# OmerMersin/video-stab

Hardware: AMD Instinct MI355X
Metric: stabilized frames/sec @1080p (whole job; warp-stage HBM GB/s in roofline) (higher is better)
Workload: dtype u8

## Files before the change

video-stab_amd/csrc/k_lk.hip:

```cpp
#include "vs_common.h"

namespace vsd {
namespace {

constexpr int MAX_LEVELS = 8;

struct LKArgs {
    LKLevel levels[MAX_LEVELS];
    int max_level;
    const float* prev_pts;
    float* next_pts;
    uint8_t* status;
    float* err;
    int n;
    const int32_t* d_n;
    int win;
    int max_count;
    double eps2;
};

template <int CTRL>
__device__ __forceinline__ int dpp_mov(int v) {
    return __builtin_amdgcn_update_dpp(0, v, CTRL, 0xF, 0xF, true);
}
__device__ __forceinline__ int wave_sum_i32(int v) {
    v += dpp_mov<0xB1>(v);
    v += dpp_mov<0x4E>(v);
    v += dpp_mov<0x141>(v);
    v += dpp_mov<0x140>(v);
    return __builtin_amdgcn_readlane(v, 0) + __builtin_amdgcn_readlane(v, 16) +
           __builtin_amdgcn_readlane(v, 32) + __builtin_amdgcn_readlane(v, 48);
}
template <int CTRL>
__device__ __forceinline__ long long dpp_mov64(long long v) {
    const int lo = dpp_mov<CTRL>((int)(unsigned)(unsigned long long)v);
    const int hi = dpp_mov<CTRL>((int)((unsigned long long)v >> 32));
    return (long long)(((unsigned long long)(unsigned)hi << 32) | (unsigned)lo);
}
__device__ __forceinline__ long long wave_sum(int p) {
    long long v = p;
    v += dpp_mov64<0xB1>(v);
    v += dpp_mov64<0x4E>(v);
    v += dpp_mov64<0x141>(v);
    v += dpp_mov64<0x140>(v);
    const int lo = (int)(unsigned)(unsigned long long)v, hi = (int)((unsigned long long)v >> 32);
    long long t = 0;
#pragma unroll
    for (int r = 0; r < 64; r += 16) {
        const unsigned l = (unsigned)__builtin_amdgcn_readlane(lo, r);
        const unsigned h = (unsigned)__builtin_amdgcn_readlane(hi, r);
        t += (long long)(((unsigned long long)h << 32) | l);
    }
    return t;
}

__device__ __forceinline__ int descale(int x, int n) { return (x + (1 << (n - 1))) >> n; }

struct Weights { int w00, w01, w10, w11; };

__device__ __forceinline__ Weights make_weights(float a, float b) {
    Weights w;
    w.w00 = f_round((1.f - a) * (1.f - b) * 16384.f);
    w.w01 = f_round(a * (1.f - b) * 16384.f);
    w.w10 = f_round((1.f - a) * b * 16384.f);
    w.w11 = 16384 - w.w00 - w.w01 - w.w10;
    return w;
}

typedef const __attribute__((address_space(1))) uint8_t* gmem_u8;
__device__ __forceinline__ gmem_u8 uniform_global(const uint8_t* p) {
    const unsigned long long v = (unsigned long long)p;
    const unsigned lo = (unsigned)__builtin_amdgcn_readfirstlane((int)(unsigned)v), hi = (unsigned)__builtin_amdgcn_readfirstlane((int)(unsigned)(v >> 32));
    return (gmem_u8)(((unsigned long long)hi << 32) | lo);
}

constexpr int LK_MARGIN = 6;
constexpr int LK_WIN_MAX = 31;



__device__ __forceinline__ void divmod_small(int i, int d, float inv_d, int& q, int& r) {
    q = (int)(((float)i + 0.5f) * inv_d);
    r = i - q * d;
}

template <int NPX>
__device__ __forceinline__ void lk_track(const LKArgs& a, const int pt) {
    constexpr int WM = NPX <= 4 ? 16 : (NPX <= 7 ? 21 : LK_WIN_MAX);
    constexpr int PWM = WM + 1, RWM = WM + 1 + 2 * LK_MARGIN;
    constexpr int DR = NPX <= 7 ? 3 : 5;
    constexpr int PPM = (PWM + 2 + 3) & ~3;
    constexpr int SRM = (PWM + 1 + 3) / 4, NGM = (PWM + DR - 1) / DR;
    static_assert(SRM * NGM <= 64, "one derivative round per level");
    constexpr int PN = (PPM * (PWM + 2) + 63) / 64, RN = (RWM * RWM + 63) / 64;
    constexpr int PBYTES = (PN * 64 > PPM * (NGM * DR + 2) + 4 ? PN * 64 : PPM * (NGM * DR + 2) + 4);
    __shared__ __attribute__((aligned(16))) uint8_t pI_[4 + PBYTES];
    uint8_t* const pI = pI_ + 4;
    __shared__ __attribute__((aligned(16))) short2 pD[(PWM + 1) * PPM];
    __shared__ uint8_t region[RN * 64];
    const int lane = threadIdx.x;
    int n = a.n;
    if (a.d_n) { int dn = *a.d_n; n = dn < n ? dn : n; }
    if (pt >= n) return;
    const int win = a.win, area = win * win;
    const int PW = win + 1, PP = (PW + 2 + 3) & ~3;
    const int RW = win + 1 + 2 * LK_MARGIN;
    const float inv_pp = 1.0f / (float)PP, inv_rw = 1.0f / (float)RW, inv_win = 1.0f / (float)win;
    uint32_t off[NPX];
#pragma unroll
    for (int k = 0; k < NPX; k++) {
        const int p = lane + 64 * k;
        int yy = 0, xx = 0;
        if (p < area) divmod_small(p, win, inv_win, yy, xx);
        off[k] = (uint32_t)((yy + 1) * PP + xx + 1) | ((uint32_t)(yy * RW + xx) << 16);
    }
#define LK_VALID(k) (lane + 64 * (k) < area)
#define LK_POFF(k) ((int)(off[k] & 0xFFFFu))
#define LK_ROFF(k) ((int)(off[k] >> 16))
    int p_y0, p_x0, p_sy, p_sx, r_y0, r_x0, r_sy, r_sx;
    divmod_small(lane, PP, inv_pp, p_y0, p_x0);
    divmod_small(64, PP, inv_pp, p_sy, p_sx);
    divmod_small(lane, RW, inv_rw, r_y0, r_x0);
    divmod_small(64, RW, inv_rw, r_sy, r_sx);
    const float halfWin = (win - 1) * 0.5f;
    const float FLT_SCALE = 1.f / (1 << 20);
    const float px0 = a.prev_pts[2 * pt], py0 = a.prev_pts[2 * pt + 1];
    float outx = 0.f, outy = 0.f;
    int status = 1;
    float err = 0.f;

    for (int level = a.max_level; level >= 0; level--) {
        const LKLevel L = a.levels[level];
        const float scale = (float)(1. / (double)(1 << level));
        float prevx = px0 * scale, prevy = py0 * scale;
        if (level == a.max_level) { outx = prevx; outy = prevy; }
        else { outx = outx * 2.f; outy = outy * 2.f; }
        prevx -= halfWin; prevy -= halfWin;
        const int ipx = f_floor(prevx), ipy = f_floor(prevy);
        if (ipx < -win || ipx >= L.w || ipy < -win || ipy >= L.h) {
            if (level == 0) { status = 0; err = 0.f; }
            continue;
        }
        float cx = outx - halfWin, cy = outy - halfWin;
        int rx0 = f_floor(cx) - LK_MARGIN, ry0 = f_floor(cy) - LK_MARGIN;
        __syncthreads();
        const int pcount = PP * (PW + 2);
        if (ipx >= 1 && ipy >= 1 && ipx - 1 + PP <= L.w && ipy + PW + 1 <= L.h) {
            const gmem_u8 pbase = uniform_global(L.prev + ((size_t)(ipy - 1) * L.stride + (ipx - 1)));
            constexpr int PB_ = 10;
            int y = p_y0, x = p_x0;
#pragma unroll
            for (int k0 = 0; k0 < PN; k0 += PB_) {
                uint8_t vI[PB_];
#pragma unroll
                for (int k = k0; k < k0 + PB_ && k < PN; k++) {
                    const bool ok = lane + 64 * k < pcount;
                    vI[k - k0] = pbase[ok ? (uint32_t)(y * (int)L.stride + x) : 0u];
                    x += p_sx; y += p_sy;
                    if (x >= PP) { x -= PP; y++; }
                }
#pragma unroll
                for (int k = k0; k < k0 + PB_ && k < PN; k++) pI[lane + 64 * k] = vI[k - k0];
                __builtin_amdgcn_sched_barrier(0);
            }
        } else {
            int y = p_y0, x = p_x0;
            for (int i = lane; i < pcount; i += 64) {
                const int X = ipx - 1 + x, Y = ipy - 1 + y;
                pI[i] = L.prev[(size_t)reflect101(Y, L.h) * L.stride + reflect101(X, L.w)];
                x += p_sx; y += p_sy;
                if (x >= PP) { x -= PP; y++; }
            }
        }
        auto stage_region = [&]() {
            const bool inside = rx0 >= 0 && ry0 >= 0 && rx0 + RW <= L.w && ry0 + RW <= L.h;
            int y = r_y0, x = r_x0;
            asm volatile("" : "+v"(x), "+v"(y));
            if (inside) {
                const gmem_u8 rbase = uniform_global(L.next + ((size_t)ry0 * L.stride + rx0));
                constexpr int RB_ = 10;
#pragma unroll
                for (int k0 = 0; k0 < RN; k0 += RB_) {
                    uint8_t vR[RB_];
#pragma unroll
                    for (int k = k0; k < k0 + RB_ && k < RN; k++) {
                        const bool ok = lane + 64 * k < RW * RW;
                        vR[k - k0] = rbase[ok ? (uint32_t)(y * (int)L.stride + x) : 0u];
                        x += r_sx; y += r_sy;
                        if (x >= RW) { x -= RW; y++; }
                    }
#pragma unroll
                    for (int k = k0; k < k0 + RB_ && k < RN; k++) region[lane + 64 * k] = vR[k - k0];
                    __builtin_amdgcn_sched_barrier(0);
                }
            } else {
                for (int i = lane; i < RW * RW; i += 64) {
                    const int X = rx0 + x, Y = ry0 + y;
                    region[i] = L.next[(size_t)reflect101(Y, L.h) * L.stride + reflect101(X, L.w)];
                    x += r_sx; y += r_sy;
                    if (x >= RW) { x -= RW; y++; }
                }
            }
        };
        stage_region();
        __syncthreads();
        {
            const int sr = (PW + 1 + 3) >> 2;
            int g, c;
            divmod_small(lane, sr, 1.0f / (float)sr, g, c);
            const int y = 1 + g * DR, x = 4 * c;
            if (y <= PW) {
                const bool masked = !(ipx >= 0 && ipy >= 0 && ipx + PW <= L.w && ipy + PW <= L.h);
                int t[3][6];
                auto load_row = [&](int j, int* tj) {
                    const uint32_t* q = reinterpret_cast<const uint32_t*>(pI + j * PP) + c;
                    const uint32_t lo = q[-1], mid = q[0], hi = q[1];
                    tj[0] = lo >> 24;
                    tj[1] = mid & 255u; tj[2] = (mid >> 8) & 255u; tj[3] = (mid >> 16) & 255u; tj[4] = mid >> 24;
                    tj[5] = hi & 255u;
                };
                load_row(y - 1, t[0]);
                load_row(y, t[1]);
#pragma unroll
                for (int r = 0; r < DR; r++) {
                    const int* t0 = t[r % 3];
                    const int* t1 = t[(r + 1) % 3];
                    int* t2 = t[(r + 2) % 3];
                    load_row(y + r + 1, t2);
                    int av[6], bv[6];
#pragma unroll
                    for (int k = 0; k < 6; k++) {
                        av[k] = (t0[k] + t2[k]) * 3 + t1[k] * 10;
                        bv[k] = t2[k] - t0[k];
                    }
                    uint32_t o[4];
#pragma unroll
                    for (int k = 0; k < 4; k++) {
                        const int dx = av[k + 2] - av[k], dy = (bv[k + 2] + bv[k]) * 3 + bv[k + 1] * 10;
                        o[k] = ((uint32_t)dx & 0xFFFFu) | ((uint32_t)dy << 16);
                        if (masked && ((unsigned)(ipx - 1 + x + k) >= (unsigned)L.w || (unsigned)(ipy - 1 + y + r) >= (unsigned)L.h)) o[k] = 0u;
                    }
                    if (y + r <= PW) *reinterpret_cast<uint4*>(&pD[(y + r) * PP + x]) = make_uint4(o[0], o[1], o[2], o[3]);
                    __builtin_amdgcn_sched_barrier(0);
                }
            }
        }
        __syncthreads();
#pragma unroll
        for (int k = 0; k < NPX; k++) asm volatile("" : "+v"(off[k]));
        Weights wt = make_weights(prevx - ipx, prevy - ipy);
        short Iw[NPX], Ix[NPX], Iy[NPX];
        int pA11 = 0, pA12 = 0, pA22 = 0;
#pragma unroll
        for (int k = 0; k < NPX; k++) {
            const int o = LK_POFF(k);
            int ival = descale(__mul24((int)pI[o], wt.w00) + __mul24((int)pI[o + 1], wt.w01) +
                               __mul24((int)pI[o + PP], wt.w10) + __mul24((int)pI[o + PP + 1], wt.w11), 9);
            const short2 d00 = pD[o], d01 = pD[o + 1], d10 = pD[o + PP], d11 = pD[o + PP + 1];
            int ixval = descale(__mul24((int)d00.x, wt.w00) + __mul24((int)d01.x, wt.w01) +
                                __mul24((int)d10.x, wt.w10) + __mul24((int)d11.x, wt.w11), 14);
            int iyval = descale(__mul24((int)d00.y, wt.w00) + __mul24((int)d01.y, wt.w01) +
                                __mul24((int)d10.y, wt.w10) + __mul24((int)d11.y, wt.w11), 14);
            if (!LK_VALID(k)) { ival = 0; ixval = 0; iyval = 0; }
            Iw[k] = (short)ival; Ix[k] = (short)ixval; Iy[k] = (short)iyval;
            pA11 += __mul24(ixval, ixval);
            pA12 += __mul24(ixval, iyval);
            pA22 += __mul24(iyval, iyval);
        }
        const long long sA11 = wave_sum(pA11), sA12 = wave_sum(pA12), sA22 = wave_sum(pA22);
        const float A11 = (float)sA11 * FLT_SCALE, A12 = (float)sA12 * FLT_SCALE, A22 = (float)sA22 * FLT_SCALE;
        float D = A11 * A22 - A12 * A12;
        const float minEig = (A22 + A11 - sqrtf((A11 - A22) * (A11 - A22) + 4.f * A12 * A12)) /
                             (float)(2 * win * win);
        if (minEig < 1e-4f || D < FLT_EPSILON) {
            if (level == 0) status = 0;
            continue;
        }
        D = 1.f / D;
        float pdx = 0.f, pdy = 0.f;
        for (int j = 0; j < a.max_count; j++) {
            const int inx = f_floor(cx), iny = f_floor(cy);
            if (inx < -win || inx >= L.w || iny < -win || iny >= L.h) {
                if (level == 0) status = 0;
                break;
            }
            wt = make_weights(cx - inx, cy - iny);
            int lx = inx - rx0, ly = iny - ry0;
            if (!(lx >= 0 && ly >= 0 && lx + win + 1 <= RW && ly + win + 1 <= RW)) {
                __syncthreads();
                rx0 = inx - LK_MARGIN; ry0 = iny - LK_MARGIN;
                stage_region();
                __syncthreads();
                lx = LK_MARGIN; ly = LK_MARGIN;
            }
            int pb1 = 0, pb2 = 0;
            {
                const int rbase = ly * RW + lx;
#pragma unroll
                for (int k = 0; k < NPX; k++) {
                    const uint8_t* r0 = &region[rbase + LK_ROFF(k)];
                    const int v = descale(__mul24((int)r0[0], wt.w00) + __mul24((int)r0[1], wt.w01) +
                                          __mul24((int)r0[RW], wt.w10) + __mul24((int)r0[RW + 1], wt.w11), 9);
                    const int diff = v - Iw[k];
                    pb1 += __mul24(diff, (int)Ix[k]);
                    pb2 += __mul24(diff, (int)Iy[k]);
                }
            }
            const long long sb1 = wave_sum(pb1), sb2 = wave_sum(pb2);
            const float b1 = (float)sb1 * FLT_SCALE, b2 = (float)sb2 * FLT_SCALE;
            const float dx = (A12 * b2 - A22 * b1) * D;
            const float dy = (A12 * b1 - A11 * b2) * D;
            cx += dx; cy += dy;
            outx = cx + halfWin; outy = cy + halfWin;
            if ((double)dx * (double)dx + (double)dy * (double)dy <= a.eps2) break;
            if (j > 0 && (double)fabsf(dx + pdx) < 0.01 && (double)fabsf(dy + pdy) < 0.01) {
                outx -= dx * 0.5f; outy -= dy * 0.5f;
                break;
            }
            pdx = dx; pdy = dy;
        }
        if (status && level == 0) {
            const float npx = outx - halfWin, npy = outy - halfWin;
            const int inx = f_floor(npx), iny = f_floor(npy);
            if (inx < -win || inx >= L.w || iny < -win || iny >= L.h) {
                status = 0;
            } else {
                wt = make_weights(npx - inx, npy - iny);
                int lx = inx - rx0, ly = iny - ry0;
                if (!(lx >= 0 && ly >= 0 && lx + win + 1 <= RW && ly + win + 1 <= RW)) {
                    __syncthreads();
                    rx0 = inx - LK_MARGIN; ry0 = iny - LK_MARGIN;
                    stage_region();
                    __syncthreads();
                    lx = LK_MARGIN; ly = LK_MARGIN;
                }
                int es = 0;
                {
                    const int rbase = ly * RW + lx;
#pragma unroll
                    for (int k = 0; k < NPX; k++) {
                        const uint8_t* r0 = &region[rbase + LK_ROFF(k)];
                        const int v = descale(__mul24((int)r0[0], wt.w00) + __mul24((int)r0[1], wt.w01) +
                                              __mul24((int)r0[RW], wt.w10) + __mul24((int)r0[RW + 1], wt.w11), 9);
                        const int diff = v - Iw[k];
                        es += LK_VALID(k) ? (diff < 0 ? -diff : diff) : 0;
                    }
                }
                const long long est = wave_sum(es);
                err = (float)est * 1.f / (float)(32 * win * win);
            }
        }
    }
#undef LK_VALID
#undef LK_POFF
#undef LK_ROFF
    if (lane == 0) {
        a.next_pts[2 * pt] = outx;
        a.next_pts[2 * pt + 1] = outy;
        a.status[pt] = (uint8_t)status;
        a.err[pt] = err;
    }
}

template <int NPX>
__global__ __launch_bounds__(64) void lk_kernel(LKArgs a) { lk_track<NPX>(a, blockIdx.x); }

template <int NPX>
__global__ __launch_bounds__(64) void lk_batch_kernel(const LKArgs* __restrict__ table) {
    lk_track<NPX>(table[blockIdx.y], blockIdx.x);
}

int fill_lk_args(LKArgs& a, const LKLevel* levels, int max_level, const float* d_prev_pts, int n, const int32_t* d_n,
                 float* d_next_pts, uint8_t* d_status, float* d_err, int win, int max_iters, double eps) {
    if (!levels || max_level < 0 || max_level >= MAX_LEVELS || n < 0 || win < 3 || win > 31 ||
        !d_prev_pts || !d_next_pts || !d_status || !d_err) {
        set_last_error("pyr_lk: invalid argument (3 <= win <= 31, max_level < 8)");
        return VS_ERR_INVALID_ARG;
    }
    for (int i = 0; i <= max_level; i++) a.levels[i] = levels[i];
    for (int i = max_level + 1; i < MAX_LEVELS; i++) a.levels[i] = levels[max_level];
    a.max_level = max_level;
    a.prev_pts = d_prev_pts; a.next_pts = d_next_pts; a.status = d_status; a.err = d_err;
    a.n = n; a.d_n = d_n; a.win = win;
    a.max_count = max_iters < 0 ? 0 : (max_iters > 100 ? 100 : max_iters);
    double e = eps < 0 ? 0. : (eps > 10. ? 10. : eps);
    a.eps2 = e * e;
    return VS_OK;
}

}

size_t lk_item_bytes() { return sizeof(LKArgs); }

int lk_fill_item(void* host_item, const LKLevel* levels, int max_level, const float* d_prev_pts, int n,
                 const int32_t* d_n, float* d_next_pts, uint8_t* d_status, float* d_err, int win, int max_iters,
                 double eps) {
    return fill_lk_args(*static_cast<LKArgs*>(host_item), levels, max_level, d_prev_pts, n, d_n, d_next_pts, d_status,
                        d_err, win, max_iters, eps);
}

int launch_pyr_lk_batch(const void* d_table, int items, int n_max, int win, hipStream_t st) {
    if (!d_table || items < 1 || items > 65535 || n_max < 0 || win < 3 || win > 31) {
        set_last_error("pyr_lk_batch: invalid argument");
        return VS_ERR_INVALID_ARG;
    }
    if (n_max == 0) return VS_OK;
    const LKArgs* t = static_cast<const LKArgs*>(d_table);
    const int npx = (win * win + 63) / 64;
    dim3 grid(n_max, items), block(64);
    if (npx <= 4) hipLaunchKernelGGL(lk_batch_kernel<4>, grid, block, 0, st, t);
    else if (npx <= 7) hipLaunchKernelGGL(lk_batch_kernel<7>, grid, block, 0, st, t);
    else hipLaunchKernelGGL(lk_batch_kernel<16>, grid, block, 0, st, t);
    VS_HIP_TRY(hipGetLastError());
    return VS_OK;
}

int launch_pyr_lk(const LKLevel* levels, int max_level, const float* d_prev_pts, int n,
                  const int32_t* d_n, float* d_next_pts, uint8_t* d_status, float* d_err, int win,
                  int max_iters, double eps, hipStream_t st) {
    LKArgs a;
    VS_TRY(fill_lk_args(a, levels, max_level, d_prev_pts, n, d_n, d_next_pts, d_status, d_err, win, max_iters, eps));
    if (n == 0) return VS_OK;
    const int npx = (win * win + 63) / 64;
    dim3 grid(n), block(64);
    if (npx <= 4) hipLaunchKernelGGL(lk_kernel<4>, grid, block, 0, st, a);
    else if (npx <= 7) hipLaunchKernelGGL(lk_kernel<7>, grid, block, 0, st, a);
    else hipLaunchKernelGGL(lk_kernel<16>, grid, block, 0, st, a);
    VS_HIP_TRY(hipGetLastError());
    return VS_OK;
}

int run_pyr_lk_op(const uint8_t* d_prev, const uint8_t* d_next, size_t stride, int w, int h,
                  const float* d_prev_pts, int n, float* d_next_pts, uint8_t* d_status,
                  float* d_err, int win, int max_level, int max_iters, double eps, hipStream_t st) {
    if (!d_prev || !d_next || w <= 0 || h <= 0 || max_level < 0 || max_level >= MAX_LEVELS) {
        set_last_error("pyr_lk: invalid argument");
        return VS_ERR_INVALID_ARG;
    }
    int lw[MAX_LEVELS], lh[MAX_LEVELS];
    int levels = 0;
    {
        int sw = w, sh = h;
        for (int level = 0; level <= max_level; level++) {
            lw[level] = sw; lh[level] = sh;
            levels = level;
            sw = (sw + 1) / 2; sh = (sh + 1) / 2;
            if (sw <= win || sh <= win) break;
        }
    }
    size_t img_bytes = 0;
    for (int i = 1; i <= levels; i++) img_bytes += (size_t)lw[i] * lh[i];
    uint8_t* scratch = nullptr;
    VS_HIP_TRY(hipMalloc((void**)&scratch, 2 * img_bytes + 64));
    LKLevel L[MAX_LEVELS];
    uint8_t* pp = scratch;
    uint8_t* pn = scratch + img_bytes;
    int rc = VS_OK;
    for (int i = 0; i <= levels && rc == VS_OK; i++) {
        L[i].w = lw[i]; L[i].h = lh[i];
        if (i == 0) { L[i].prev = d_prev; L[i].next = d_next; L[i].stride = stride; }
        else {
            rc = launch_pyr_down(L[i - 1].prev, L[i - 1].stride, lw[i - 1], lh[i - 1], pp, lw[i], st);
            if (rc == VS_OK) rc = launch_pyr_down(L[i - 1].next, L[i - 1].stride, lw[i - 1], lh[i - 1], pn, lw[i], st);
            L[i].prev = pp; L[i].next = pn; L[i].stride = lw[i];
            pp += (size_t)lw[i] * lh[i]; pn += (size_t)lw[i] * lh[i];
        }
    }
    if (rc == VS_OK) rc = launch_pyr_lk(L, levels, d_prev_pts, n, nullptr, d_next_pts, d_status, d_err, win, max_iters, eps, st);
    hipError_t e = hipStreamSynchronize(st);
    (void)hipFree(scratch);
    if (rc == VS_OK && e != hipSuccess) { set_last_error(hipGetErrorString(e)); rc = VS_ERR_HIP; }
    return rc;
}

}
```

Measured before the change: 127,400.

## Stage LK patches with aligned dword loads and packed 16-bit derivative math

Stages the prev patch and next search region from global memory with aligned 32-bit loads joined by alignbyte, replacing per-byte loads, and pads the region to a 4-byte pitch. The Scharr derivative computation now uses packed 16-bit SIMD arithmetic and perm/alignbit instead of scalar byte unpacking. Wave reductions do their first steps in 32-bit where the value range proves no overflow, and per-NPX VGPR limits are set on the kernels. Pyramid level buffers are padded to 4 bytes so the aligned path applies, at the cost of more complex staging code and register-pressure tuning risk.

```diff
diff --git a/video-stab_amd/csrc/k_lk.hip b/video-stab_amd/csrc/k_lk.hip
--- a/video-stab_amd/csrc/k_lk.hip
+++ b/video-stab_amd/csrc/k_lk.hip
@@ -1,4 +1,5 @@
 #include "vs_common.h"
+#include "lk_stage.h"
 
 namespace vsd {
 namespace {
@@ -31,18 +32,33 @@
     return __builtin_amdgcn_readlane(v, 0) + __builtin_amdgcn_readlane(v, 16) +
            __builtin_amdgcn_readlane(v, 32) + __builtin_amdgcn_readlane(v, 48);
 }
+constexpr long long LK_DIFF_MAX = 8161, LK_GRAD_MAX = 4081;
+constexpr long long LK_TERM_MAX = LK_DIFF_MAX * LK_GRAD_MAX;
+constexpr int lk_sum32_steps(int npx) {
+    int s = 0;
+    while (s < 4 && (long long)npx * LK_TERM_MAX * (2ll << s) <= 2147483647ll) s++;
+    return s;
+}
 template <int CTRL>
 __device__ __forceinline__ long long dpp_mov64(long long v) {
     const int lo = dpp_mov<CTRL>((int)(unsigned)(unsigned long long)v);
     const int hi = dpp_mov<CTRL>((int)((unsigned long long)v >> 32));
     return (long long)(((unsigned long long)(unsigned)hi << 32) | (unsigned)lo);
 }
+template <int NPX>
 __device__ __forceinline__ long long wave_sum(int p) {
+    constexpr int S32 = lk_sum32_steps(NPX);
+    static_assert((long long)NPX * LK_TERM_MAX <= 2147483647ll, "a lane's partial sum fits int32");
+    static_assert((long long)NPX * LK_TERM_MAX * (1ll << S32) <= 2147483647ll, "the 32-bit steps cannot overflow");
+    if (S32 >= 1) p += dpp_mov<0xB1>(p);
+    if (S32 >= 2) p += dpp_mov<0x4E>(p);
+    if (S32 >= 3) p += dpp_mov<0x141>(p);
+    if (S32 >= 4) p += dpp_mov<0x140>(p);
     long long v = p;
-    v += dpp_mov64<0xB1>(v);
-    v += dpp_mov64<0x4E>(v);
-    v += dpp_mov64<0x141>(v);
-    v += dpp_mov64<0x140>(v);
+    if (S32 < 1) v += dpp_mov64<0xB1>(v);
+    if (S32 < 2) v += dpp_mov64<0x4E>(v);
+    if (S32 < 3) v += dpp_mov64<0x141>(v);
+    if (S32 < 4) v += dpp_mov64<0x140>(v);
     const int lo = (int)(unsigned)(unsigned long long)v, hi = (int)((unsigned long long)v >> 32);
     long long t = 0;
 #pragma unroll
@@ -53,6 +69,12 @@
     }
     return t;
 }
+
+typedef unsigned short u16x2 __attribute__((ext_vector_type(2)));
+__device__ __forceinline__ uint32_t pk_add(uint32_t a, uint32_t b) { return __builtin_bit_cast(uint32_t, __builtin_bit_cast(u16x2, a) + __builtin_bit_cast(u16x2, b)); }
+__device__ __forceinline__ uint32_t pk_sub(uint32_t a, uint32_t b) { return __builtin_bit_cast(uint32_t, __builtin_bit_cast(u16x2, a) - __builtin_bit_cast(u16x2, b)); }
+__device__ __forceinline__ uint32_t pk_mul(uint32_t a, uint32_t b) { return __builtin_bit_cast(uint32_t, __builtin_bit_cast(u16x2, a) * __builtin_bit_cast(u16x2, b)); }
+__device__ __forceinline__ uint32_t pk_mad(uint32_t a, uint32_t b, uint32_t c) { return pk_add(pk_mul(a, b), c); }
 
 __device__ __forceinline__ int descale(int x, int n) { return (x + (1 << (n - 1))) >> n; }
 
@@ -68,6 +90,7 @@
 }
 
 typedef const __attribute__((address_space(1))) uint8_t* gmem_u8;
+typedef const __attribute__((address_space(1))) uint32_t* gmem_u32;
 __device__ __forceinline__ gmem_u8 uniform_global(const uint8_t* p) {
     const unsigned long long v = (unsigned long long)p;
     const unsigned lo = (unsigned)__builtin_amdgcn_readfirstlane((int)(unsigned)v), hi = (unsigned)__builtin_amdgcn_readfirstlane((int)(unsigned)(v >> 32));
@@ -93,18 +116,20 @@
     constexpr int SRM = (PWM + 1 + 3) / 4, NGM = (PWM + DR - 1) / DR;
     static_assert(SRM * NGM <= 64, "one derivative round per level");
     constexpr int PN = (PPM * (PWM + 2) + 63) / 64, RN = (RWM * RWM + 63) / 64;
+    constexpr int RPM = (RWM + 3) & ~3;
+    constexpr int PND = (PPM / 4 * (PWM + 2) + 63) / 64, RND = (RPM / 4 * RWM + 63) / 64;
     constexpr int PBYTES = (PN * 64 > PPM * (NGM * DR + 2) + 4 ? PN * 64 : PPM * (NGM * DR + 2) + 4);
     __shared__ __attribute__((aligned(16))) uint8_t pI_[4 + PBYTES];
     uint8_t* const pI = pI_ + 4;
     __shared__ __attribute__((aligned(16))) short2 pD[(PWM + 1) * PPM];
-    __shared__ uint8_t region[RN * 64];
+    __shared__ __attribute__((aligned(16))) uint8_t region[RPM * RWM];
     const int lane = threadIdx.x;
     int n = a.n;
     if (a.d_n) { int dn = *a.d_n; n = dn < n ? dn : n; }
     if (pt >= n) return;
     const int win = a.win, area = win * win;
     const int PW = win + 1, PP = (PW + 2 + 3) & ~3;
-    const int RW = win + 1 + 2 * LK_MARGIN;
+    const int RW = win + 1 + 2 * LK_MARGIN, RP = (RW + 3) & ~3;
     const float inv_pp = 1.0f / (float)PP, inv_rw = 1.0f / (float)RW, inv_win = 1.0f / (float)win;
     uint32_t off[NPX];
 #pragma unroll
@@ -112,16 +137,18 @@
         const int p = lane + 64 * k;
         int yy = 0, xx = 0;
         if (p < area) divmod_small(p, win, inv_win, yy, xx);
-        off[k] = (uint32_t)((yy + 1) * PP + xx + 1) | ((uint32_t)(yy * RW + xx) << 16);
+        off[k] = (uint32_t)((yy + 1) * PP + xx + 1) | ((uint32_t)(yy * RP + xx) << 16);
     }
 #define LK_VALID(k) (lane + 64 * (k) < area)
 #define LK_POFF(k) ((int)(off[k] & 0xFFFFu))
 #define LK_ROFF(k) ((int)(off[k] >> 16))
-    int p_y0, p_x0, p_sy, p_sx, r_y0, r_x0, r_sy, r_sx;
-    divmod_small(lane, PP, inv_pp, p_y0, p_x0);
-    divmod_small(64, PP, inv_pp, p_sy, p_sx);
-    divmod_small(lane, RW, inv_rw, r_y0, r_x0);
-    divmod_small(64, RW, inv_rw, r_sy, r_sx);
+    auto walk = [&](int d, float inv_d, int& y0, int& x0, int& sy, int& sx) {
+        int ln = lane;
+        asm volatile("" : "+v"(ln));
+        divmod_small(ln, d, inv_d, y0, x0);
+        divmod_small(64, d, inv_d, sy, sx);
+        return ln;
+    };
     const float halfWin = (win - 1) * 0.5f;
     const float FLT_SCALE = 1.f / (1 << 20);
     const float px0 = a.prev_pts[2 * pt], py0 = a.prev_pts[2 * pt + 1];
@@ -145,10 +172,33 @@
         int rx0 = f_floor(cx) - LK_MARGIN, ry0 = f_floor(cy) - LK_MARGIN;
         __syncthreads();
         const int pcount = PP * (PW + 2);
-        if (ipx >= 1 && ipy >= 1 && ipx - 1 + PP <= L.w && ipy + PW + 1 <= L.h) {
+        const bool p_inside = lk_box_inside(ipx - 1, ipy - 1, PP, PW + 2, L.w, L.h);
+        if (p_inside && (((unsigned long long)L.prev | (unsigned long long)L.stride) & 3u) == 0) {
+            const gmem_u8 pbase = uniform_global(L.prev + (size_t)(ipy - 1) * L.stride);
+            const int nd = PP >> 2, cnt = nd * (PW + 2), x0 = ipx - 1;
+            const LKStageSrc s0 = lk_stage_src(x0, PP, 0);
+            int y, j, sy, sj;
+            const int ln = walk(nd, 4.0f * inv_pp, y, j, sy, sj);
+            uint32_t vlo[PND], vhi[PND];
+#pragma unroll
+            for (int k = 0; k < PND; k++) {
+                const bool ok = ln + 64 * k < cnt;
+                const LKStageSrc sc = lk_stage_src(x0, PP, j);
+                const uint32_t row = (uint32_t)(y * (int)L.stride);
+                vlo[k] = *reinterpret_cast<gmem_u32>(pbase + (ok ? row + (uint32_t)sc.lo : (uint32_t)s0.lo));
+                vhi[k] = *reinterpret_cast<gmem_u32>(pbase + (ok ? row + (uint32_t)sc.hi : (uint32_t)s0.lo));
+                j += sj; y += sy;
+                if (j >= nd) { j -= nd; y++; }
+            }
+#pragma unroll
+            for (int k = 0; k < PND; k++)
+                if (ln + 64 * k < cnt) reinterpret_cast<uint32_t*>(pI)[ln + 64 * k] = lk_stage_join(vlo[k], vhi[k], s0.shift);
+            __builtin_amdgcn_sched_barrier(0);
+        } else if (p_inside) {
             const gmem_u8 pbase = uniform_global(L.prev + ((size_t)(ipy - 1) * L.stride + (ipx - 1)));
             constexpr int PB_ = 10;
-            int y = p_y0, x = p_x0;
+            int y, x, p_sy, p_sx;
+            walk(PP, inv_pp, y, x, p_sy, p_sx);
 #pragma unroll
             for (int k0 = 0; k0 < PN; k0 += PB_) {
                 uint8_t vI[PB_];
@@ -164,7 +214,8 @@
                 __builtin_amdgcn_sched_barrier(0);
             }
         } else {
-            int y = p_y0, x = p_x0;
+            int y, x, p_sy, p_sx;
+            walk(PP, inv_pp, y, x, p_sy, p_sx);
             for (int i = lane; i < pcount; i += 64) {
                 const int X = ipx - 1 + x, Y = ipy - 1 + y;
                 pI[i] = L.prev[(size_t)reflect101(Y, L.h) * L.stride + reflect101(X, L.w)];
@@ -173,30 +224,63 @@
             }
         }
         auto stage_region = [&]() {
-            const bool inside = rx0 >= 0 && ry0 >= 0 && rx0 + RW <= L.w && ry0 + RW <= L.h;
-            int y = r_y0, x = r_x0;
-            asm volatile("" : "+v"(x), "+v"(y));
-            if (inside) {
+            const bool inside = lk_box_inside(rx0, ry0, RW, RW, L.w, L.h);
+            if (inside && (((unsigned long long)L.next | (unsigned long long)L.stride) & 3u) == 0) {
+                const gmem_u8 rbase = uniform_global(L.next + (size_t)ry0 * L.stride);
+                const int nd = RP >> 2, cnt = nd * RW;
+                const LKStageSrc s0 = lk_stage_src(rx0, RW, 0);
+                int y, j, sy, sj;
+                const int ln = walk(nd, 1.0f / (float)nd, y, j, sy, sj);
+                constexpr int RB_ = 5;
+#pragma unroll
+                for (int k0 = 0; k0 < RND; k0 += RB_) {
+                    uint32_t vlo[RB_], vhi[RB_];
+#pragma unroll
+                    for (int k = k0; k < k0 + RB_ && k < RND; k++) {
+                        const bool ok = ln + 64 * k < cnt;
+                        const LKStageSrc sc = lk_stage_src(rx0, RW, j);
+                        const uint32_t row = (uint32_t)(y * (int)L.stride);
+                        vlo[k - k0] = *reinterpret_cast<gmem_u32>(rbase + (ok ? row + (uint32_t)sc.lo : (uint32_t)s0.lo));
+                        vhi[k - k0] = *reinterpret_cast<gmem_u32>(rbase + (ok ? row + (uint32_t)sc.hi : (uint32_t)s0.lo));
+                        j += sj; y += sy;
+                        if (j >= nd) { j -= nd; y++; }
+                    }
+#pragma unroll
+                    for (int k = k0; k < k0 + RB_ && k < RND; k++)
+                        if (ln + 64 * k < cnt)
+                            reinterpret_cast<uint32_t*>(region)[ln + 64 * k] = lk_stage_join(vlo[k - k0], vhi[k - k0], s0.shift);
+                    __builtin_amdgcn_sched_barrier(0);
+                }
+            } else if (inside) {
                 const gmem_u8 rbase = uniform_global(L.next + ((size_t)ry0 * L.stride + rx0));
-                constexpr int RB_ = 10;
+                constexpr int RB_ = 2;
+                int y, x, r_sy, r_sx;
+                const int ln = walk(RW, inv_rw, y, x, r_sy, r_sx);
 #pragma unroll
                 for (int k0 = 0; k0 < RN; k0 += RB_) {
                     uint8_t vR[RB_];
+                    int ys = y, xs = x;
 #pragma unroll
                     for (int k = k0; k < k0 + RB_ && k < RN; k++) {
-                        const bool ok = lane + 64 * k < RW * RW;
+                        const bool ok = ln + 64 * k < RW * RW;
                         vR[k - k0] = rbase[ok ? (uint32_t)(y * (int)L.stride + x) : 0u];
                         x += r_sx; y += r_sy;
                         if (x >= RW) { x -= RW; y++; }
                     }
 #pragma unroll
-                    for (int k = k0; k < k0 + RB_ && k < RN; k++) region[lane + 64 * k] = vR[k - k0];
+                    for (int k = k0; k < k0 + RB_ && k < RN; k++) {
+                        if (ln + 64 * k < RW * RW) region[ys * RP + xs] = vR[k - k0];
+                        xs += r_sx; ys += r_sy;
+                        if (xs >= RW) { xs -= RW; ys++; }
+                    }
                     __builtin_amdgcn_sched_barrier(0);
                 }
             } else {
+                int y, x, r_sy, r_sx;
+                walk(RW, inv_rw, y, x, r_sy, r_sx);
                 for (int i = lane; i < RW * RW; i += 64) {
                     const int X = rx0 + x, Y = ry0 + y;
-                    region[i] = L.next[(size_t)reflect101(Y, L.h) * L.stride + reflect101(X, L.w)];
+                    region[y * RP + x] = L.next[(size_t)reflect101(Y, L.h) * L.stride + reflect101(X, L.w)];
                     x += r_sx; y += r_sy;
                     if (x >= RW) { x -= RW; y++; }
                 }
@@ -211,35 +295,39 @@
             const int y = 1 + g * DR, x = 4 * c;
             if (y <= PW) {
                 const bool masked = !(ipx >= 0 && ipy >= 0 && ipx + PW <= L.w && ipy + PW <= L.h);
-                int t[3][6];
-                auto load_row = [&](int j, int* tj) {
+                static_assert(16 * 255 <= 32767, "smoothing sums and derivatives fit a signed 16-bit half");
+                uint32_t t[3][3];
+                auto load_row = [&](int j, uint32_t* tj) {
                     const uint32_t* q = reinterpret_cast<const uint32_t*>(pI + j * PP) + c;
                     const uint32_t lo = q[-1], mid = q[0], hi = q[1];
-                    tj[0] = lo >> 24;
-                    tj[1] = mid & 255u; tj[2] = (mid >> 8) & 255u; tj[3] = (mid >> 16) & 255u; tj[4] = mid >> 24;
-                    tj[5] = hi & 255u;
+                    tj[0] = __builtin_amdgcn_perm(mid, lo, 0x0c040c03u);
+                    tj[1] = __builtin_amdgcn_perm(mid, mid, 0x0c020c01u);
+                    tj[2] = __builtin_amdgcn_perm(hi, mid, 0x0c040c03u);
                 };
                 load_row(y - 1, t[0]);
                 load_row(y, t[1]);
 #pragma unroll
                 for (int r = 0; r < DR; r++) {
-                    const int* t0 = t[r % 3];
-                    const int* t1 = t[(r + 1) % 3];
-                    int* t2 = t[(r + 2) % 3];
+                    const uint32_t* t0 = t[r % 3];
+                    const uint32_t* t1 = t[(r + 1) % 3];
+                    uint32_t* t2 = t[(r + 2) % 3];
                     load_row(y + r + 1, t2);
-                    int av[6], bv[6];
-#pragma unroll
-                    for (int k = 0; k < 6; k++) {
-                        av[k] = (t0[k] + t2[k]) * 3 + t1[k] * 10;
-                        bv[k] = t2[k] - t0[k];
+                    uint32_t av[3], bv[3];
+#pragma unroll
+                    for (int k = 0; k < 3; k++) {
+                        av[k] = pk_mad(pk_add(t0[k], t2[k]), 0x00030003u, pk_mul(t1[k], 0x000a000au));
+                        bv[k] = pk_sub(t2[k], t0[k]);
                     }
+                    const uint32_t bq0 = __builtin_amdgcn_alignbit(bv[1], bv[0], 16), bq1 = __builtin_amdgcn_alignbit(bv[2], bv[1], 16);
+                    const uint32_t dx0 = pk_sub(av[1], av[0]), dx1 = pk_sub(av[2], av[1]);
+                    const uint32_t dy0 = pk_mad(pk_add(bv[0], bv[1]), 0x00030003u, pk_mul(bq0, 0x000a000au));
+                    const uint32_t dy1 = pk_mad(pk_add(bv[1], bv[2]), 0x00030003u, pk_mul(bq1, 0x000a000au));
                     uint32_t o[4];
-#pragma unroll
-                    for (int k = 0; k < 4; k++) {
-                        const int dx = av[k + 2] - av[k], dy = (bv[k + 2] + bv[k]) * 3 + bv[k + 1] * 10;
-                        o[k] = ((uint32_t)dx & 0xFFFFu) | ((uint32_t)dy << 16);
+                    o[0] = __builtin_amdgcn_perm(dy0, dx0, 0x05040100u); o[1] = __builtin_amdgcn_perm(dy0, dx0, 0x07060302u);
+                    o[2] = __builtin_amdgcn_perm(dy1, dx1, 0x05040100u); o[3] = __builtin_amdgcn_perm(dy1, dx1, 0x07060302u);
+#pragma unroll
+                    for (int k = 0; k < 4; k++)
                         if (masked && ((unsigned)(ipx - 1 + x + k) >= (unsigned)L.w || (unsigned)(ipy - 1 + y + r) >= (unsigned)L.h)) o[k] = 0u;
-                    }
                     if (y + r <= PW) *reinterpret_cast<uint4*>(&pD[(y + r) * PP + x]) = make_uint4(o[0], o[1], o[2], o[3]);
                     __builtin_amdgcn_sched_barrier(0);
                 }
@@ -267,7 +355,7 @@
             pA12 += __mul24(ixval, iyval);
             pA22 += __mul24(iyval, iyval);
         }
-        const long long sA11 = wave_sum(pA11), sA12 = wave_sum(pA12), sA22 = wave_sum(pA22);
+        const long long sA11 = wave_sum<NPX>(pA11), sA12 = wave_sum<NPX>(pA12), sA22 = wave_sum<NPX>(pA22);
         const float A11 = (float)sA11 * FLT_SCALE, A12 = (float)sA12 * FLT_SCALE, A22 = (float)sA22 * FLT_SCALE;
         float D = A11 * A22 - A12 * A12;
         const float minEig = (A22 + A11 - sqrtf((A11 - A22) * (A11 - A22) + 4.f * A12 * A12)) /
@@ -295,18 +383,18 @@
             }
             int pb1 = 0, pb2 = 0;
             {
-                const int rbase = ly * RW + lx;
+                const int rbase = ly * RP + lx;
 #pragma unroll
                 for (int k = 0; k < NPX; k++) {
                     const uint8_t* r0 = &region[rbase + LK_ROFF(k)];
                     const int v = descale(__mul24((int)r0[0], wt.w00) + __mul24((int)r0[1], wt.w01) +
-                                          __mul24((int)r0[RW], wt.w10) + __mul24((int)r0[RW + 1], wt.w11), 9);
+                                          __mul24((int)r0[RP], wt.w10) + __mul24((int)r0[RP + 1], wt.w11), 9);
                     const int diff = v - Iw[k];
                     pb1 += __mul24(diff, (int)Ix[k]);
                     pb2 += __mul24(diff, (int)Iy[k]);
                 }
             }
-            const long long sb1 = wave_sum(pb1), sb2 = wave_sum(pb2);
+            const long long sb1 = wave_sum<NPX>(pb1), sb2 = wave_sum<NPX>(pb2);
             const float b1 = (float)sb1 * FLT_SCALE, b2 = (float)sb2 * FLT_SCALE;
             const float dx = (A12 * b2 - A22 * b1) * D;
             const float dy = (A12 * b1 - A11 * b2) * D;
@@ -336,17 +424,17 @@
                 }
                 int es = 0;
                 {
-                    const int rbase = ly * RW + lx;
+                    const int rbase = ly * RP + lx;
 #pragma unroll
                     for (int k = 0; k < NPX; k++) {
                         const uint8_t* r0 = &region[rbase + LK_ROFF(k)];
                         const int v = descale(__mul24((int)r0[0], wt.w00) + __mul24((int)r0[1], wt.w01) +
-                                              __mul24((int)r0[RW], wt.w10) + __mul24((int)r0[RW + 1], wt.w11), 9);
+                                              __mul24((int)r0[RP], wt.w10) + __mul24((int)r0[RP + 1], wt.w11), 9);
                         const int diff = v - Iw[k];
                         es += LK_VALID(k) ? (diff < 0 ? -diff : diff) : 0;
                     }
                 }
-                const long long est = wave_sum(es);
+                const long long est = wave_sum<NPX>(es);
                 err = (float)est * 1.f / (float)(32 * win * win);
             }
         }
@@ -362,13 +450,20 @@
     }
 }
 
-template <int NPX>
-__global__ __launch_bounds__(64) void lk_kernel(LKArgs a) { lk_track<NPX>(a, blockIdx.x); }
-
-template <int NPX>
-__global__ __launch_bounds__(64) void lk_batch_kernel(const LKArgs* __restrict__ table) {
-    lk_track<NPX>(table[blockIdx.y], blockIdx.x);
-}
+template <int NPX> __global__ void lk_kernel(LKArgs a);
+template <int NPX> __global__ void lk_batch_kernel(const LKArgs* __restrict__ table);
+#define LK_KERNELS(NPX, VGPRS)                                                                                              \
+    template <> __global__ __launch_bounds__(64) __attribute__((amdgpu_num_vgpr(VGPRS))) void lk_kernel<NPX>(LKArgs a) {     \
+        lk_track<NPX>(a, blockIdx.x);                                                                                       \
+    }                                                                                                                       \
+    template <> __global__ __launch_bounds__(64) __attribute__((amdgpu_num_vgpr(VGPRS)))                                     \
+    void lk_batch_kernel<NPX>(const LKArgs* __restrict__ table) {                                                           \
+        lk_track<NPX>(table[blockIdx.y], blockIdx.x);                                                                       \
+    }
+LK_KERNELS(4, 96)
+LK_KERNELS(7, 120)
+LK_KERNELS(16, 208)
+#undef LK_KERNELS
 
 int fill_lk_args(LKArgs& a, const LKLevel* levels, int max_level, const float* d_prev_pts, int n, const int32_t* d_n,
                  float* d_next_pts, uint8_t* d_status, float* d_err, int win, int max_iters, double eps) {
@@ -448,8 +543,9 @@
             if (sw <= win || sh <= win) break;
         }
     }
+    auto level_bytes = [&](int i) { return ((size_t)lw[i] * lh[i] + 3) & ~(size_t)3; };
     size_t img_bytes = 0;
-    for (int i = 1; i <= levels; i++) img_bytes += (size_t)lw[i] * lh[i];
+    for (int i = 1; i <= levels; i++) img_bytes += level_bytes(i);
     uint8_t* scratch = nullptr;
     VS_HIP_TRY(hipMalloc((void**)&scratch, 2 * img_bytes + 64));
     LKLevel L[MAX_LEVELS];
@@ -463,7 +559,7 @@
             rc = launch_pyr_down(L[i - 1].prev, L[i - 1].stride, lw[i - 1], lh[i - 1], pp, lw[i], st);
             if (rc == VS_OK) rc = launch_pyr_down(L[i - 1].next, L[i - 1].stride, lw[i - 1], lh[i - 1], pn, lw[i], st);
             L[i].prev = pp; L[i].next = pn; L[i].stride = lw[i];
-            pp += (size_t)lw[i] * lh[i]; pn += (size_t)lw[i] * lh[i];
+            pp += level_bytes(i); pn += level_bytes(i);
         }
     }
     if (rc == VS_OK) rc = launch_pyr_lk(L, levels, d_prev_pts, n, nullptr, d_next_pts, d_status, d_err, win, max_iters, eps, st);
diff --git a/video-stab_amd/csrc/lk_stage.h b/video-stab_amd/csrc/lk_stage.h
--- /dev/null
+++ b/video-stab_amd/csrc/lk_stage.h
@@ -0,0 +1,46 @@
+#pragma once
+#include <stdint.h>
+
+#if defined(__HIPCC__)
+#define LKS_HD __host__ __device__
+#else
+#define LKS_HD
+#endif
+
+namespace vsd {
+
+LKS_HD inline int lk_stage_dwords(int cols) { return (cols + 3) >> 2; }
+
+LKS_HD inline bool lk_box_inside(int x0, int y0, int cols, int rows, int w, int h) {
+    return x0 >= 0 && y0 >= 0 && x0 + cols <= w && y0 + rows <= h;
+}
+
+LKS_HD inline bool lk_stage_fast(uint64_t base, uint64_t pitch, int x0, int y0, int cols, int rows, int w, int h) {
+    return ((base | pitch) & 3u) == 0 && lk_box_inside(x0, y0, cols, rows, w, h);
+}
+
+struct LKStageSrc {
+    int lo, hi;
+    int shift;
+};
+
+LKS_HD inline LKStageSrc lk_stage_src(int x0, int cols, int j) {
+    const int b = x0 + 4 * j, last = (x0 + cols - 1) & ~3;
+    LKStageSrc s;
+    s.shift = b & 3;
+    s.lo = b & ~3;
+    s.hi = s.lo + 4 < last ? s.lo + 4 : last;
+    return s;
+}
+
+LKS_HD inline int lk_stage_lds(int y, int j, int nd) { return 4 * (y * nd + j); }
+
+LKS_HD inline uint32_t lk_stage_join(uint32_t lo, uint32_t hi, int shift) {
+#if defined(__HIP_DEVICE_COMPILE__)
+    return __builtin_amdgcn_alignbyte(hi, lo, (uint32_t)shift);
+#else
+    return (uint32_t)(((((uint64_t)hi) << 32) | lo) >> (8 * shift));
+#endif
+}
+
+}
```

Result: no change. 128,800, median of 4 (+1.1%).
